# kkaytekin/Supervised-Depth-Estimation-from-Polarized-Images

Measured on AMD Instinct MI355X. Metric: train images/sec (512x612, 3-encoder), higher is better.
Workload: dtype f32; 1 GPU; BASELINE configs[2]: full 3-encoder (augment_xolp+augment_normals), multi-scale loss scales=[0,1,2,3], batch 16 per GPU, 512x612 frames (network/loss on 512x640 padded), dropout 0.1, Adam lr 1e-4, fp32; global_batch=16, height=512, width=640, frame_width=612, parallelism=dp1

## Files before the change

### include/polardepth.h

```cpp
#ifndef POLARDEPTH_H
#define POLARDEPTH_H

#include <stddef.h>
#include <stdint.h>

#ifdef __cplusplus
extern "C" {
#endif

#define PD_OK 0
#define PD_EINVAL (-22)
#define PD_ELAUNCH (-5)

const char* pd_last_error(void);
int pd_version(void);

#define PD_POLAR_LS 0
#define PD_POLAR_STOKES 1
#define PD_POLAR_PRECISE_NORMALS 1
#define PD_POLAR_IEEE_RHO 2
#define PD_POLAR_NT_LOADS 4
#define PD_POLAR_PLAIN_LOADS 8

size_t pd_polar_tables_bytes(int n_d, int n_s1, int n_s2);
int pd_polar_tables_pack(const double* x_d, const double* y_d, int n_d,
                         const double* x_s1, const double* y_s1, int n_s1,
                         const double* x_s2, const double* y_s2, int n_s2,
                         void* host_blob, size_t blob_bytes);
int pd_polar_tables_build(double n, void* host_blob, size_t blob_bytes, size_t* blob_bytes_used);

int pd_polar_fwd(const void* pol, const void* mask, void* xolp, void* xolp_std, void* normals,
                 void* ints, const void* tables, size_t tables_bytes,
                 int B, int H, int W, int Wout, int mode, int flags, void* stream);

int pd_polar_normals_from_xolp(const void* xolp, void* normals, const void* tables, size_t tables_bytes,
                               int B, int H, int W, int flags, void* stream);

int pd_polar_calc_normals(const void* phi, const void* theta, void* out, int B, long P, int phi_f64, int theta_f64,
                          void* stream);

int pd_polar_theta(const void* rho, void* theta_d, void* theta_s1, void* theta_s2, void* bins,
                   const void* tables, size_t tables_bytes, long n, void* stream);

int pd_polar_fit_matrix(const double angles_rad[4], double coef_out[12]);

#define PD_POLAR_U8 0
#define PD_POLAR_U16 1
#define PD_POLAR_F32 2
int pd_polar_general_fwd(const void* pol, int dtype, const double* coef, void* iun, void* xolp, void* xolp_std,
                         void* normals, const void* tables, size_t tables_bytes,
                         int B, int H, int W, int Wout, int flags, void* stream);

#define PD_XOLP_STATS_BYTES 4184
size_t pd_xolp_stats_workspace(int B, int H, int W);
int pd_xolp_stats(const void* xolp, const void* mask, void* stats, void* workspace, size_t ws_bytes,
                  int B, int H, int W, int ld, const float thresholds[2], int accumulate, void* stream);

#define PD_CONV_AUTO 0u
#define PD_CONV_FP32_MFMA 1u
#define PD_CONV_BF16X3 2u
#define PD_CONV_WGRAD_SPLIT_IN_REGS 4u
#define PD_CONV_GENERAL_KERNELS 8u
#define PD_CONV_X3_IM2COL 16u
#define PD_CONV_WGRAD_ROW_WORKGROUPS 32u
#define PD_CONV_BF16 128u
#define PD_CONV_FLAGS_ALL 191u
int pd_conv2d_tile_m(long M, int Cout);
long pd_conv2d_stats_rows(long M, int Cout);
int pd_conv2d_uses_x3(long M, int Cout, int C, int KH, int KW, int stride, int pad, int mode, int act, int has_out_scale,
                      int Ho, int Wo, unsigned flags);
int pd_conv2d_uses_bf16(long M, int Cout, int C, int KH, int KW, int stride, int pad, int mode, int act, int has_out_scale,
                        int Ho, int Wo, unsigned flags);
int pd_conv2d_route(long M, int Cout, int C, int KH, int KW, int stride, int pad, int mode, int act, int has_out_scale,
                    int Ho, int Wo, unsigned flags);
int pd_conv2d(const void* x, const void* w, const void* bias, const void* out_scale, void* y, void* stats,
              int N, int H, int W, int C, long sN, long sH, long sW, long sC,
              int Ho, int Wo, int Cout, int KH, int KW, int stride, int pad, int mode, int act,
              int affine, float sub, float div, long ldy, unsigned flags, void* stream);

int pd_conv16(const void* x, const void* w, const void* bias, void* y, int N, int H, int W, int C,
              long sN, long sH, long sW, int Ho, int Wo, int Cout, long ldy, int mode, int act, void* stream);

size_t pd_conv16_wgrad_workspace(int C);
int pd_conv16_wgrad(const void* x, const void* dz, void* dw, void* dbias, void* workspace, size_t ws_bytes,
                    int N, int H, int W, int C, long sN, long sH, long sW, long ldd, int accumulate, void* stream);

int pd_dgrad_s2_filters(const void* wt, void* wsub, int Cin, int Cout, void* stream);
int pd_conv2d_rect(const void* x, const void* w, void* y, int N, int H, int W, int C, long sN, long sH, long sW, long sC,
                   int Ho, int Wo, int Cout, int KH, int KW, int pad_h, int pad_w, int mode, long ldy, unsigned flags,
                   void* stream);
int pd_interleave4(const void* sub, void* dx, int N, int Ho, int Wo, int C, void* stream);

int pd_conv2d_add(const void* x, const void* w, const void* addend, long ld_add, void* y,
                  int N, int H, int W, int C, long sN, long sH, long sW, long sC,
                  int Ho, int Wo, int Cout, int KH, int KW, int stride, int pad, int mode, long ldy, unsigned flags,
                  void* stream);

size_t pd_conv2d_wgrad_workspace(long M, int Cout, int K, unsigned flags);
int pd_conv2d_wgrad(const void* x, const void* dy, void* dw, void* dbias, void* workspace, size_t ws_bytes,
                    int N, int H, int W, int C, long sN, long sH, long sW, long sC,
                    int Ho, int Wo, int Cout, int KH, int KW, int stride, int pad, int mode,
                    int affine, float sub, float div, long ldd, int accumulate, unsigned flags, void* stream);
int pd_conv2d_wgrad_uses_x3(long M, int Cout, int C, int KH, int KW, int stride, int pad, int mode, int H, int W, int Ho, int Wo,
                            unsigned flags);
int pd_conv2d_wgrad_uses_bf16(long M, int Cout, int C, int KH, int KW, int stride, int pad, int mode, int H, int W, int Ho, int Wo,
                              unsigned flags);

int pd_stem_s2d_input(const void* x, void* out, int N, int C, int H, int W, long sN, long sC, long sH, long sW,
                      int affine, float sub, float div, void* stream);
int pd_stem_s2d_weight(const void* w, void* w2, int Cout, int C, void* stream);
int pd_stem_s2d_weight_grad(const void* dw2, void* dw, int Cout, int C, int accumulate, void* stream);

int pd_weight_transpose(const void* w, void* wt, int Cout, int T, int Cin, void* stream);
int pd_weight_transpose_batched(const void* src, void* dst, const void* table, const void* blk, int n, int nblocks,
                                void* stream);

int pd_bn_fwd_finalize(const void* partial, long R, int C, double count, const void* gamma, const void* beta,
                       void* running_mean, void* running_var, float momentum, float eps, void* acc_ws, long acc_len,
                       void* scale, void* shift, void* save_mean, void* save_invstd, int training, void* stream);
int pd_bn_bwd_finalize(const void* partial, long R, int C, double count, void* acc_ws, long acc_len, void* dgamma,
                       void* dbeta, void* coef, int accumulate, void* stream);
long pd_chain_bwd_rows(int N, int H, int W, int C);
int pd_chain_fwd(const void* x, const void* scale, const void* shift, const void* res, void* out,
                 int N, int H, int W, int C, long ld_res, long ld_out, int relu_pre, int pool,
                 float drop_p, uint64_t seed, uint64_t offset, const void* step_state, int relu_post, void* stream);
int pd_chain_bwd_reduce(const void* dy, long ld_dy, const void* x, const void* out, long ld_out,
                        const void* scale, const void* shift, const void* mean, const void* invstd,
                        void* partial, int N, int H, int W, int C, int relu_pre, int pool, float drop_p,
                        uint64_t seed, uint64_t offset, const void* step_state, int relu_post, void* stream);
int pd_chain_bwd_apply(const void* dy, long ld_dy, const void* x, const void* out, long ld_out,
                       const void* scale, const void* shift, const void* mean, const void* invstd,
                       const void* coef, void* dx, void* dres, int N, int H, int W, int C, int relu_pre,
                       int pool, float drop_p, uint64_t seed, uint64_t offset, const void* step_state, int relu_post,
                       void* stream);

int pd_maxpool3s2_fwd(const void* x, void* y, void* idx, int N, int H, int W, int C, void* stream);
int pd_maxpool3s2_bwd(const void* idx, const void* dy, void* dx, int N, int H, int W, int C, void* stream);
int pd_maxpool3s2_bwd_add(const void* idx, const void* dy, const void* addend, long ld_add, void* dx, int N, int H, int W,
                          int C, void* stream);

int pd_upcat_fwd(const void* a, const void* skip, long ld_skip, void* out, int N, int H, int W, int Ca, int Cs,
                 void* stream);
int pd_up_bwd(const void* dout, long ld_d, void* da, int N, int H, int W, int Ca, void* stream);
int pd_up_bwd_elu(const void* dout, long ld_d, const void* elu_y, void* da, int N, int H, int W, int Ca, void* stream);

int pd_up2x_ac_fwd(const void* a, void* out, int N, int H, int W, int C, void* stream);
int pd_up2x_ac_bwd(const void* dout, void* da, int N, int H, int W, int C, void* stream);
int pd_relu_add(const void* x, const void* res, void* out, long n, int relu, void* stream);

// ... 139 lines not shown
```

### supervised-depth-estimation-from-polarized-images_amd/csrc/conv.hip

```cpp
#include "pd_common.h"
#include <cstdlib>
#include <type_traits>

namespace {

typedef float f32x16 __attribute__((ext_vector_type(16)));
typedef unsigned int u32x4 __attribute__((ext_vector_type(4)));

constexpr int BK = 32;
constexpr int LDT = BK;
constexpr int NT = 256;
constexpr unsigned OOB = 0x80000000u;

enum { MODE_ZERO = 0, MODE_REFLECT = 1, MODE_TRANSPOSED = 2 };
enum { ACT_NONE = 0, ACT_RELU = 1, ACT_ELU = 2, ACT_SIGMOID = 3 };

#define PD_I(n) std::integral_constant<int, n>{}
#define PD_SB __builtin_amdgcn_sched_barrier(0);

template <typename F> void with_mode(int mode, F&& f) {
    if (mode == MODE_ZERO) f(PD_I(MODE_ZERO)); else if (mode == MODE_REFLECT) f(PD_I(MODE_REFLECT)); else f(PD_I(MODE_TRANSPOSED));
}
template <typename F> void with_bool(bool b, F&& f) { if (b) f(std::true_type{}); else f(std::false_type{}); }

// ... 1980 lines not shown
        auto mm = [&](const x3::Terms& t, auto g_tag, auto n_tag) {
            constexpr int G = decltype(g_tag)::value, N = decltype(n_tag)::value, T = N / 2, BLK = N % 2;
            const unsigned* bv = T < 3 ? t.h : T < 5 ? t.m : t.l;
            const u32x4 av = T == 0 ? fa[G][BLK][0] : T == 1 ? fa[G][BLK][1] : T == 2 ? fa[G][BLK][2] : T == 3 ? fa[G][BLK][0] : T == 4 ? fa[G][BLK][1] : fa[G][BLK][0];
            acc[BLK] = __builtin_amdgcn_mfma_f32_32x32x16_bf16(bf(av), bf(u32x4{bv[0], bv[1], bv[2], bv[3]}), acc[BLK], 0, 0, 0);
        };
        x3::sp_h<0>(x0, t0); x3::sp_h<1>(x0, t0); x3::sp_h<2>(x0, t0); x3::sp_h<3>(x0, t0);
        PD_SB
#define PD_XP(j) if constexpr (SPREAD) load_x_piece(nxt, PD_I(j));
#define PD_DP(j) if constexpr (SPREAD) load_d_piece(buf_tag, PD_I(j));
        mm(t0, PD_I(0), PD_I(0)); x3::sp_m<0>(x0, t0); PD_XP(0) PD_SB
        mm(t0, PD_I(0), PD_I(1)); x3::sp_m<1>(x0, t0); PD_XP(1) PD_SB
        mm(t0, PD_I(0), PD_I(2)); x3::sp_m<2>(x0, t0); PD_XP(2) PD_SB
        mm(t0, PD_I(0), PD_I(3)); x3::sp_m<3>(x0, t0); PD_XP(3) PD_SB
        mm(t0, PD_I(0), PD_I(4)); x3::sp_h<0>(dv, td); x3::sp_h<1>(dv, td); x3::sp_h<2>(dv, td); x3::sp_h<3>(dv, td); PD_DP(0) PD_SB
        mm(t0, PD_I(0), PD_I(5)); x3::sp_m<0>(dv, td); PD_DP(1) PD_SB
#undef PD_XP
#undef PD_DP
        mm(t0, PD_I(0), PD_I(6)); x3::sp_l<0>(t0); x3::sp_h<0>(x1, t1); PD_SB
        mm(t0, PD_I(0), PD_I(7)); x3::sp_l<1>(t0); x3::sp_h<1>(x1, t1); PD_SB
        mm(t0, PD_I(0), PD_I(8)); x3::sp_l<2>(t0); x3::sp_h<2>(x1, t1); PD_SB
        mm(t0, PD_I(0), PD_I(9)); x3::sp_l<3>(t0); x3::sp_h<3>(x1, t1); PD_SB
        mm(t0, PD_I(0), PD_I(10)); x3::sp_m<1>(dv, td); PD_SB
        mm(t0, PD_I(0), PD_I(11)); x3::sp_m<2>(dv, td); PD_SB
        mm(t1, PD_I(1), PD_I(0)); x3::sp_m<0>(x1, t1); PD_SB
        mm(t1, PD_I(1), PD_I(1)); x3::sp_m<1>(x1, t1); PD_SB
        mm(t1, PD_I(1), PD_I(2)); x3::sp_m<2>(x1, t1); PD_SB
        mm(t1, PD_I(1), PD_I(3)); x3::sp_m<3>(x1, t1); PD_SB
        mm(t1, PD_I(1), PD_I(4)); x3::sp_m<3>(dv, td); PD_SB
        mm(t1, PD_I(1), PD_I(5)); x3::sp_l<0>(td); x3::sp_l<1>(td); PD_SB
        mm(t1, PD_I(1), PD_I(6)); x3::sp_l<0>(t1); PD_SB
        mm(t1, PD_I(1), PD_I(7)); x3::sp_l<1>(t1); PD_SB
        mm(t1, PD_I(1), PD_I(8)); x3::sp_l<2>(t1); PD_SB
        mm(t1, PD_I(1), PD_I(9)); x3::sp_l<3>(t1); PD_SB
        mm(t1, PD_I(1), PD_I(10)); x3::sp_l<2>(td); x3::sp_l<3>(td); PD_SB
        mm(t1, PD_I(1), PD_I(11));
        if constexpr (BIAS) bsum += ((dv[0] + dv[1]) + (dv[2] + dv[3])) + ((dv[4] + dv[5]) + (dv[6] + dv[7]));
        *reinterpret_cast<u32x4*>(lds_c + sp_off + (NXT * P_BYTES + 0 * 4096u)) = u32x4{td.h[0], td.h[1], td.h[2], td.h[3]};
        *reinterpret_cast<u32x4*>(lds_c + sp_off + (NXT * P_BYTES + 1 * 4096u)) = u32x4{td.m[0], td.m[1], td.m[2], td.m[3]};
        *reinterpret_cast<u32x4*>(lds_c + sp_off + (NXT * P_BYTES + 2 * 4096u)) = u32x4{td.l[0], td.l[1], td.l[2], td.l[3]};
        dma_wait();
        __syncthreads();
    };

    {
        const std::integral_constant<unsigned, 0> d0{};
        const std::integral_constant<unsigned, 1> d1{};
        load_x_all(d0);
        load_d(d0);
        load_d(d1);
        dma_wait();
        __syncthreads();
        split_d(d0);
        __syncthreads();
    }
    for (int q = 0; q < nchunks; q += 2) {
        chunk(std::integral_constant<unsigned, 0>{});
        if (q + 1 < nchunks) chunk(std::integral_constant<unsigned, 1>{});
        if ((q & (FLUSH - 2)) == FLUSH - 2) flush();
    }
    flush();

#pragma unroll
    for (int blk = 0; blk < 2; ++blk) {
        const int k = k0 + wave * 32 + fi;
#pragma unroll
        for (int r = 0; r < 16; ++r) {
            const int co = co0 + 32 * blk + (r & 3) + 8 * (r >> 2) + 4 * fk;
            if (co < a.Co && k < a.K) a.part[((long)s * a.Co + co) * a.K + k] = acc_sum[blk][r];
        }
    }
    if constexpr (BIAS) {
        if (do_bias) {
            float* red = smem_all;
            red[wave * 64 + lane] = bsum;
            __syncthreads();
            if (tid < 64 && co0 + tid < a.Co) a.bpart[(long)s * a.Co + co0 + tid] = (red[tid] + red[64 + tid]) + (red[128 + tid] + red[192 + tid]);
        }
    }
}

#include "conv_wgrad_halo.hpp"
#include "conv_wgrad_roll.hpp"

__global__ __launch_bounds__(256) void reduce_rows_kernel(const float* __restrict__ part, float* __restrict__ out,
                                                          int S, long n, int accumulate) {
    __shared__ float red[4][64];
    const int col = threadIdx.x & 63, sl = threadIdx.x >> 6;
    const long i = blockIdx.x * 64L + col;
    float a0 = 0.f, a1 = 0.f, a2 = 0.f, a3 = 0.f;
    if (i < n) {
        int j = sl;
        for (; j + 12 < S; j += 16) {
            a0 += part[(long)j * n + i];
            a1 += part[(long)(j + 4) * n + i];
            a2 += part[(long)(j + 8) * n + i];
            a3 += part[(long)(j + 12) * n + i];
        }
        for (; j < S; j += 4) a0 += part[(long)j * n + i];
    }
    red[sl][col] = (a0 + a1) + (a2 + a3);
    __syncthreads();
    if (sl == 0 && i < n) {
        const float s = (red[0][col] + red[1][col]) + (red[2][col] + red[3][col]);
        out[i] = accumulate ? out[i] + s : s;
    }
}

__global__ __launch_bounds__(256) void weight_transpose_kernel(const float* __restrict__ w, float* __restrict__ wt,
                                                               int Co, int T, int Ci) {
    const long n = (long)Co * T * Ci;
    for (long i = blockIdx.x * 256L + threadIdx.x; i < n; i += (long)gridDim.x * 256) {
        const int co = (int)(i % Co);
        const long r = i / Co;
        const int t = (int)(r % T);
        const int ci = (int)(r / T);
        wt[i] = w[((long)co * T + t) * Ci + ci];
    }
}

__global__ __launch_bounds__(256) void weight_transpose_batched_kernel(const float* __restrict__ src, float* __restrict__ dst,
                                                                       const int* __restrict__ table,
                                                                       const int* __restrict__ blk, int n) {
    __shared__ float tile[32][33];
    int lo = 0, hi = n;
    while (hi - lo > 1) {
        const int mid = (lo + hi) >> 1;
        if (blk[mid] <= (int)blockIdx.x) lo = mid; else hi = mid;
    }
    const int off = table[4 * lo], Co = table[4 * lo + 1], T = table[4 * lo + 2], Ci = table[4 * lo + 3];
    const float* w = src + off;
    float* wt = dst + off;
    int lb = (int)blockIdx.x - blk[lo];
    const int tiles_ci = (Ci + 31) >> 5, tiles_co = (Co + 31) >> 5;
    const int ci0 = (lb % tiles_ci) << 5; lb /= tiles_ci;
    const int co0 = (lb % tiles_co) << 5;
    const int t = lb / tiles_co;
    const int x = threadIdx.x & 31, y = threadIdx.x >> 5;
#pragma unroll
    for (int r = y; r < 32; r += 8)
        if (co0 + r < Co && ci0 + x < Ci) tile[r][x] = w[((long)(co0 + r) * T + t) * Ci + ci0 + x];
    __syncthreads();
#pragma unroll
    for (int r = y; r < 32; r += 8)
        if (ci0 + r < Ci && co0 + x < Co) wt[((long)(ci0 + r) * T + t) * Co + co0 + x] = tile[x][r];
}

inline int wgrad_tco(int Co) { return Co > 32 ? 64 : (Co > 16 ? 32 : 16); }

inline bool wgrad_x3c_enabled(unsigned flags) { return !(flags & (PD_CONV_FP32_MFMA | PD_CONV_WGRAD_SPLIT_IN_REGS)); }
inline bool wgrad_x3_on(unsigned flags) { return (flags & PD_CONV_WGRAD_SPLIT_IN_REGS) && !(flags & PD_CONV_FP32_MFMA); }

void wgrad_plan(long M, int Co, int K, unsigned flags, int* S, long* mper) {
    const int tco = wgrad_tco(Co);
    const long tiles = (long)((Co + tco - 1) / tco) * ((K + WG_K - 1) / WG_K);
    const bool x3c = tco == 64 && wgrad_x3c_enabled(flags) && !(flags & PD_CONV_GENERAL_KERNELS);
    const long total = x3c ? (512 / tiles < 4 ? 1536 : M >= (1L << 20) ? 1024 : 512) : (tiles <= 32 ? 768 : 1536);
    long s = total / tiles;
    const long smax = (M + 511) / 512;
    if (s > smax) s = smax;
    if (s < 1) s = 1;
    long per = (M + s - 1) / s;
    per = (per + WG_MC - 1) / WG_MC * WG_MC;
    s = (M + per - 1) / per;
    if (s < 1) s = 1;
    *S = (int)s; *mper = per;
}

enum WgradFamily { WGRAD_GENERAL = 0, WGRAD_UNI, WGRAD_UNI_X3, WGRAD_X3C, WGRAD_HALO, WGRAD_ROLL };
struct WgradRoute {
    int family;
    int tco, S; long mper;
    bool vec, row8;
    int nb, nbw;
    int s_cap; bool bf16;
    WgradRollPlan roll;
};

static WgradRoute route_wgrad(const WgradArgs& a, bool vec, unsigned flags, size_t ws_bytes) {
    WgradRoute r{};
    r.vec = vec; r.tco = wgrad_tco(a.Co);
    wgrad_plan(a.M, a.Co, a.K, flags, &r.S, &r.mper);
    const bool refl_ok = a.mode == MODE_REFLECT && a.pad == 1 && a.KH == 3 && a.KW == 3 && a.stride == 1 && a.Ho == a.H && a.Wo == a.W && a.H >= 3;
    if (!(a.mode == MODE_ZERO || refl_ok)) return r;
    if (wgrad_x3c_enabled(flags) && !(flags & (PD_CONV_GENERAL_KERNELS | PD_CONV_X3_IM2COL)) && wgrad_halo_eligible(a, vec)) {
        r.bf16 = (flags & PD_CONV_BF16) != 0;
        const size_t per_slice = ((size_t)a.Co * a.K + a.Co) * sizeof(float);
        r.s_cap = (int)std::min<size_t>((r.bf16 ? pd_conv2d_wgrad_workspace(a.M, a.Co, a.K, flags) : ws_bytes) / per_slice, 1 << 20);
        r.family = !(flags & PD_CONV_WGRAD_ROW_WORKGROUPS) && wgrad_roll_eligible(a, vec, r.s_cap, r.roll) ? WGRAD_ROLL : WGRAD_HALO;
        return r;
    }
    r.nb = (a.pad + a.stride - 1) / a.stride; r.nbw = (r.nb + 1) / 2;
    if (!(flags & PD_CONV_GENERAL_KERNELS) && (r.tco == 64 || r.tco == 32) && vec && a.Co % 4 == 0 && a.Wo % 2 == 0 && a.ldd % 4 == 0 &&
        a.Ho >= 2 * r.nb && a.Wo >= 4 * r.nbw && a.Wo >= 14 && (2 * r.nb + 1) * (2 * r.nbw + 1) <= 31 && r.mper % WG_MC == 0 &&
        a.M % 4 == 0 && a.K >= 4) {
        r.family = r.tco == 32 ? WGRAD_UNI : wgrad_x3c_enabled(flags) ? WGRAD_X3C : wgrad_x3_on(flags) ? WGRAD_UNI_X3 : WGRAD_UNI;
        r.row8 = a.Wo % 8 == 0 && r.mper % 8 == 0 && a.M % 8 == 0;
    }
    return r;
}

static int launch_wgrad_slices(const WgradArgs& a, const WgradRoute& r, bool bias, hipStream_t st) {
    const dim3 grid((unsigned)(((long)a.ktiles * a.ctiles * a.S + 7) / 8 * 8)), block(NT);
    const bool reflect = a.mode == MODE_REFLECT;
    if (r.family == WGRAD_GENERAL) {
        const auto gen = [&](auto tco) { with_bool(r.vec, [&](auto v) { with_bool(reflect, [&](auto refl) {
            hipLaunchKernelGGL((conv_wgrad_kernel<decltype(tco)::value, decltype(v)::value, decltype(refl)::value ? MODE_REFLECT : MODE_ZERO>), grid, block, 0, st, a);
        }); }); };
        if (r.tco == 64) gen(PD_I(64)); else if (r.tco == 32) gen(PD_I(32)); else gen(PD_I(16));
        return PD_OK;
    }
    WgradUniArgs ua; ua.g = a; ua.nb = r.nb; ua.nbw = r.nbw;
    if (r.family == WGRAD_X3C) {
        static const hipError_t lds_ok = [] {
            hipError_t e = hipSuccess;
            for (const void* f : {reinterpret_cast<const void*>(conv_wgrad_x3c_kernel<true, true>), reinterpret_cast<const void*>(conv_wgrad_x3c_kernel<false, true>),
                                  reinterpret_cast<const void*>(conv_wgrad_x3c_kernel<true, false>), reinterpret_cast<const void*>(conv_wgrad_x3c_kernel<false, false>),
                                  reinterpret_cast<const void*>(conv_wgrad_x3c_kernel<true, false, true>), reinterpret_cast<const void*>(conv_wgrad_x3c_kernel<false, false, true>)}) {
                const hipError_t rc = hipFuncSetAttribute(f, hipFuncAttributeMaxDynamicSharedMemorySize, x3c::LDS_BYTES);
                if (rc != hipSuccess) e = rc;
            }
            return e;
        }();
        PD_REQUIRE(lds_ok == hipSuccess, "pd_conv2d_wgrad: cannot reserve %u bytes of LDS", x3c::LDS_BYTES);
        with_bool(bias, [&](auto b) {
            constexpr bool B = decltype(b)::value;
            if (reflect) hipLaunchKernelGGL((conv_wgrad_x3c_kernel<B, false, true>), grid, block, x3c::LDS_BYTES, st, ua);
            else if (r.row8) hipLaunchKernelGGL((conv_wgrad_x3c_kernel<B, true>), grid, block, x3c::LDS_BYTES, st, ua);
            else hipLaunchKernelGGL((conv_wgrad_x3c_kernel<B, false>), grid, block, x3c::LDS_BYTES, st, ua);
        });
    } else if (r.tco == 32) {
        with_bool(reflect, [&](auto refl) { hipLaunchKernelGGL((conv_wgrad_uni_kernel<decltype(refl)::value, true, 32>), grid, block, 0, st, ua); });
    } else {
        with_bool(reflect, [&](auto refl) { with_bool(bias, [&](auto b) {
            constexpr bool R = decltype(refl)::value, B = decltype(b)::value;
            if (r.family == WGRAD_UNI_X3) hipLaunchKernelGGL((conv_wgrad_uni_kernel<R, B, 64, true>), grid, block, 0, st, ua);
            else hipLaunchKernelGGL((conv_wgrad_uni_kernel<R, B>), grid, block, 0, st, ua);
        }); });
    }
    return PD_OK;
}

static void fill_wgrad_args(WgradArgs& a, int N, int H, int W, int C, long sN, long sH, long sW, long sC, int Ho, int Wo, int Co,
                            int KH, int KW, int stride, int pad, int mode, int affine, float sub, float div, long ldd) {
    a.N = N; a.H = H; a.W = W; a.C = C; a.sN = sN; a.sH = sH; a.sW = sW; a.sC = sC;
    a.Ho = Ho; a.Wo = Wo; a.Co = Co; a.KH = KH; a.KW = KW; a.stride = stride; a.pad = pad; a.mode = mode;
    a.affine = affine; a.sub = sub; a.div = div;
    a.K = KH * KW * C; a.M = (long)N * Ho * Wo; a.ldd = ldd;
}

}

extern "C" size_t pd_conv2d_wgrad_workspace(long M, int Co, int K, unsigned flags) {
    int S; long mper;
    wgrad_plan(M, Co, K, flags, &S, &mper);
    if (wgrad_x3c_enabled(flags) && !(flags & (PD_CONV_GENERAL_KERNELS | PD_CONV_X3_IM2COL))) {
        const int sh = std::max(wgrad_halo_slices_bound(Co, K), wgrad_roll_slices_bound(Co, K));
        const long cap = (M + 63) / 64;
        S = S > (sh < cap ? sh : (int)cap) ? S : (sh < cap ? sh : (int)cap);
    }
    return ((size_t)S * Co * K + (size_t)S * Co) * sizeof(float);
}

extern "C" int pd_conv2d_wgrad_uses_x3(long M, int Co, int C, int KH, int KW, int stride, int pad, int mode, int H, int W, int Ho,
                                       int Wo, unsigned flags) {
    if (Ho <= 0 || Wo <= 0) return 0;
    WgradArgs a{};
    fill_wgrad_args(a, (int)(M / ((long)Ho * Wo)), H, W, C, (long)H * W * C, (long)W * C, C, 1, Ho, Wo, Co, KH, KW, stride, pad, mode,
                    0, 0.f, 1.f, Co);
    a.M = M;
    const int family = route_wgrad(a, vec16_ok(a.x, C, a.sN, a.sH, a.sW, a.sC, a.affine), flags, pd_conv2d_wgrad_workspace(M, Co, a.K, flags)).family;
    return family == WGRAD_ROLL ? 3 : family == WGRAD_HALO ? 2 : family == WGRAD_X3C ? 1 : 0;
}

extern "C" int pd_conv2d_wgrad_uses_bf16(long M, int Co, int C, int KH, int KW, int stride, int pad, int mode, int H, int W, int Ho,
                                         int Wo, unsigned flags) {
    if (!(flags & PD_CONV_BF16) || !pd::conv_flags_ok(flags)) return 0;
    const int r = pd_conv2d_wgrad_uses_x3(M, Co, C, KH, KW, stride, pad, mode, H, W, Ho, Wo, flags);
    return r >= 2 ? r : 0;
}

extern "C" int pd_conv2d_wgrad(const void* x, const void* dy, void* dw, void* dbias, void* workspace, size_t ws_bytes,
                               int N, int H, int W, int C, long sN, long sH, long sW, long sC,
                               int Ho, int Wo, int Co, int KH, int KW, int stride, int pad, int mode,
                               int affine, float sub, float div, long ldd, int accumulate, unsigned flags, void* stream) {
    PD_REQUIRE(x && dy && dw && workspace, "pd_conv2d_wgrad: null tensor");
    PD_REQUIRE(pd::conv_flags_ok(flags), "pd_conv2d_wgrad: bad flags 0x%x", flags);
    PD_REQUIRE(mode == MODE_ZERO || mode == MODE_REFLECT, "pd_conv2d_wgrad: mode must be 0 or 1");
    PD_REQUIRE(Ho <= (H + 2 * pad - KH) / stride + 1 && Wo <= (W + 2 * pad - KW) / stride + 1,
               "pd_conv2d_wgrad: output grid does not match input/filter geometry");
    PD_REQUIRE(ldd >= Co && (ldd % 4 == 0 || Co < 4) , "pd_conv2d_wgrad: bad dy row stride");
    if (N == 0) return PD_OK;
    WgradArgs a;
    a.x = (const float*)x; a.dy = (const float*)dy;
    fill_wgrad_args(a, N, H, W, C, sN, sH, sW, sC, Ho, Wo, Co, KH, KW, stride, pad, mode, affine, sub, div, ldd);
    const size_t need = pd_conv2d_wgrad_workspace(a.M, Co, a.K, flags);
    PD_REQUIRE(ws_bytes >= need, "pd_conv2d_wgrad: workspace too small (%zu < %zu)", ws_bytes, need);
    PD_REQUIRE(pd::aligned16(dy) && (ldd % 4 == 0 || Co < 4), "pd_conv2d_wgrad: dy must be 16-byte aligned rows");
    const WgradRoute r = route_wgrad(a, vec16_ok(x, C, sN, sH, sW, sC, affine), flags, ws_bytes);
    a.S = r.S; a.mper = r.mper;
    PD_REQUIRE(a.mper * ldd * 4 < 0x7fffffffL, "pd_conv2d_wgrad: slice too large for 32-bit offsets");
    PD_REQUIRE((a.mper / ((long)Ho * Wo) + 2) * sN * 4 < 0x7fffffffL, "pd_conv2d_wgrad: image too large for 32-bit offsets");
    a.part = (float*)workspace;
    a.bpart = dbias ? a.part + (size_t)a.S * Co * a.K : nullptr;
    a.ktiles = (a.K + WG_K - 1) / WG_K; a.ctiles = (Co + r.tco - 1) / r.tco;
    hipStream_t st = (hipStream_t)stream;
    int S = a.S;
    if (r.family == WGRAD_ROLL) S = launch_wgrad_roll(a, r.roll, st, dbias != nullptr, r.bf16);
    else if (r.family == WGRAD_HALO) S = launch_wgrad_halo(a, r.s_cap, st, dbias != nullptr, r.bf16);
    else if (int rc = launch_wgrad_slices(a, r, dbias != nullptr, st)) return rc;
    a.bpart = dbias ? a.part + (size_t)S * Co * a.K : nullptr;
    if (int rc = pd::check_launch("pd_conv2d_wgrad")) return rc;
    const long nw = (long)Co * a.K;
    hipLaunchKernelGGL(reduce_rows_kernel, dim3((unsigned)((nw + 63) / 64)), dim3(256), 0, st, a.part, (float*)dw, S, nw, accumulate);
    if (dbias)
        hipLaunchKernelGGL(reduce_rows_kernel, dim3((unsigned)((Co + 63) / 64)), dim3(256), 0, st, a.bpart, (float*)dbias, S, (long)Co, accumulate);
    return pd::check_launch("pd_conv2d_wgrad/reduce");
}

extern "C" int pd_weight_transpose(const void* w, void* wt, int Co, int T, int Ci, void* stream) {
    PD_REQUIRE(w && wt && Co > 0 && T > 0 && Ci > 0, "pd_weight_transpose: bad arguments");
    const long n = (long)Co * T * Ci;
    const long blocks = (n + 255) / 256;
    hipLaunchKernelGGL(weight_transpose_kernel, dim3((unsigned)(blocks > 4096 ? 4096 : blocks)), dim3(256), 0,
                       (hipStream_t)stream, (const float*)w, (float*)wt, Co, T, Ci);
    return pd::check_launch("pd_weight_transpose");
}

extern "C" int pd_weight_transpose_batched(const void* src, void* dst, const void* table, const void* blk, int n,
                                           int nblocks, void* stream) {
    PD_REQUIRE(src && dst && table && blk && n > 0 && nblocks > 0, "pd_weight_transpose_batched: bad arguments");
    hipLaunchKernelGGL(weight_transpose_batched_kernel, dim3((unsigned)nblocks), dim3(256), 0, (hipStream_t)stream,
                       (const float*)src, (float*)dst, (const int*)table, (const int*)blk, n);
    return pd::check_launch("pd_weight_transpose_batched");
}

namespace {
__global__ __launch_bounds__(256) void dgrad_s2_filters_kernel(const float* __restrict__ wt, float* __restrict__ wsub,
                                                               int Ci, int Co) {
    const long cc = (long)Ci * Co, total = 9 * cc;
    for (long i = blockIdx.x * 256L + threadIdx.x; i < total; i += (long)gridDim.x * 256) {
        const int cls = i < cc ? 0 : i < 3 * cc ? 1 : i < 5 * cc ? 2 : 3, ph = cls >> 1, pw = cls & 1;
        const long base = cc * (cls == 0 ? 0 : cls == 1 ? 1 : cls == 2 ? 3 : 5);
        long r = i - base;
        const int co = (int)(r % Co); r /= Co;
        const int kw2 = pw ? (int)(r & 1) : 0; r >>= pw;
        const int kh2 = ph ? (int)(r & 1) : 0; r >>= ph;
        const int ci = (int)r;
        const int kh = ph ? (kh2 ? 2 : 0) : 1, kw = pw ? (kw2 ? 2 : 0) : 1;
        wsub[i] = wt[(((long)ci * 3 + kh) * 3 + kw) * Co + co];
    }
}
__global__ __launch_bounds__(256) void interleave4_kernel(const float* __restrict__ sub, float* __restrict__ dx, int N, int Ho,
                                                          int Wo, int C) {
    const int cq = C >> 2;
    const long per = (long)N * Ho * Wo * cq, total = 4 * per;
    for (long i = blockIdx.x * 256L + threadIdx.x; i < total; i += (long)gridDim.x * 256) {
        const int c4 = (int)(i % cq) * 4;
        long r = i / cq;
        const int pw = (int)(r & 1); r >>= 1;
        const int j = (int)(r % Wo); r /= Wo;
        const int ph = (int)(r & 1); r >>= 1;
        const int ii = (int)(r % Ho);
        const long n = r / Ho;
        const float4 v = ldg4(sub + ((long)(ph * 2 + pw) * N * Ho * Wo + (n * Ho + ii) * (long)Wo + j) * C + c4);
        *reinterpret_cast<float4*>(dx + ((n * 2 * Ho + 2 * ii + ph) * (long)(2 * Wo) + 2 * j + pw) * C + c4) = v;
    }
}
}

extern "C" int pd_dgrad_s2_filters(const void* wt, void* wsub, int Ci, int Co, void* stream) {
    PD_REQUIRE(wt && wsub && Ci > 0 && Co > 0, "pd_dgrad_s2_filters: bad arguments");
    const long total = 9L * Ci * Co, blocks = (total + 255) / 256;
    hipLaunchKernelGGL(dgrad_s2_filters_kernel, dim3((unsigned)(blocks > 2048 ? 2048 : blocks)), dim3(256), 0,
                       (hipStream_t)stream, (const float*)wt, (float*)wsub, Ci, Co);
    return pd::check_launch("pd_dgrad_s2_filters");
}

extern "C" int pd_interleave4(const void* sub, void* dx, int N, int Ho, int Wo, int C, void* stream) {
    PD_REQUIRE(sub && dx && N > 0 && Ho > 0 && Wo > 0 && C > 0 && C % 4 == 0, "pd_interleave4: bad arguments");
    const long total = 4L * N * Ho * Wo * (C / 4), blocks = (total + 255) / 256;
    hipLaunchKernelGGL(interleave4_kernel, dim3((unsigned)(blocks > 8192 ? 8192 : blocks)), dim3(256), 0,
                       (hipStream_t)stream, (const float*)sub, (float*)dx, N, Ho, Wo, C);
    return pd::check_launch("pd_interleave4");
}

namespace {

__global__ __launch_bounds__(256) void s2d_input_kernel(const float* __restrict__ x, float* __restrict__ out, int N,
                                                        int C, int H, int W, long sN, long sC, long sH, long sW,
                                                        int affine, float sub, float div) {
    const int H2 = H >> 1, W2 = W >> 1, C4 = 4 * C;
// ... 99 lines not shown
```

### supervised-depth-estimation-from-polarized-images_amd/polardepth/ops.py

```python
import os

import torch

from ._lib import lib, check, ptr, stream_ptr

MODE_ZERO, MODE_REFLECT, MODE_TRANSPOSED = 0, 1, 2
ACT_NONE, ACT_RELU, ACT_ELU, ACT_SIGMOID = 0, 1, 2, 3
CL = torch.channels_last
PROFILE = None

CONV_AUTO, CONV_FP32_MFMA, CONV_BF16X3, CONV_WGRAD_SPLIT_IN_REGS, CONV_GENERAL_KERNELS, CONV_X3_IM2COL = 0, 1, 2, 4, 8, 16
CONV_WGRAD_ROW_WORKGROUPS = 32
CONV_BF16 = 128
CONV_FLAGS = (CONV_FP32_MFMA if os.environ.get("PD_CONV_X3", "1") == "0" else
              CONV_X3_IM2COL if os.environ.get("PD_CONV_HALO", "1") == "0" else CONV_AUTO)
WGRAD_FLAGS = (CONV_FP32_MFMA if os.environ.get("PD_WGRAD_X3C", "1") == "0" else
               CONV_X3_IM2COL if os.environ.get("PD_CONV_HALO", "1") == "0" else
               CONV_WGRAD_ROW_WORKGROUPS if os.environ.get("PD_WGRAD_ROLL", "1") == "0" else CONV_AUTO)


class conv_flags:

    def __init__(self, conv=None, wgrad=None):
        self.new = (conv, wgrad)

    def __enter__(self):
        global CONV_FLAGS, WGRAD_FLAGS
        self.old = (CONV_FLAGS, WGRAD_FLAGS)
        if self.new[0] is not None:
            CONV_FLAGS = int(self.new[0])
        if self.new[1] is not None:
            WGRAD_FLAGS = int(self.new[1])
        return self

    def __exit__(self, *exc):
        global CONV_FLAGS, WGRAD_FLAGS
        CONV_FLAGS, WGRAD_FLAGS = self.old
        return False


def conv_bf16_mode():
    return (bool(CONV_FLAGS & CONV_BF16), bool(WGRAD_FLAGS & CONV_BF16))


def _with_bf16(word, bf16):
    if bf16 is None:
        return word
    if bf16 and not (word & (CONV_FP32_MFMA | CONV_BF16X3)):
        return word | CONV_BF16
    return word & ~CONV_BF16


def _profiled(label, flops, fn, shape=None):
    if PROFILE is None:
        return fn()
    e0, e1 = torch.cuda.Event(enable_timing=True), torch.cuda.Event(enable_timing=True)
    e0.record()
    r = fn()
    e1.record()
    PROFILE.append((label, flops, e0, e1, shape))
    return r


_IGEMM_LABELS = ("conv_igemm_kernel<{bm},{bn},{gather}>", "conv_igemm_uni_kernel<{bm},{bn}>", "conv_igemm_x3_kernel<{bm},{bn}>",
                 "conv_halo_x3_kernel<8x32,64>", "conv_halo_bf16_kernel<8x32,64>")


def _igemm_label(M, Co, vec, kind, C=0, KH=1, KW=1, stride=1, pad=0, mode=0, act=ACT_NONE, out_scale=False, out_hw=(0, 0),
                 flags=None):
    flags = CONV_FLAGS if flags is None else flags
    if not vec:
        flags = CONV_FP32_MFMA | CONV_GENERAL_KERNELS
    r = lib.pd_conv2d_route(M, Co, C, KH, KW, stride, pad, mode, act, int(out_scale), out_hw[0], out_hw[1], flags)
    return _IGEMM_LABELS[r & 15].format(bm=r >> 12, bn=(r >> 4) & 255, gather="vec" if vec else "scalar")


def _require_cuda(*ts):
    for t in ts:
        if t is not None and not t.is_cuda:
            raise RuntimeError("polardepth ops need CUDA(HIP) tensors; there is no CPU fallback")


def empty_nhwc(n, c, h, w, device):
    return torch.empty((n, c, h, w), dtype=torch.float32, device=device, memory_format=CL)


def is_nhwc(t):
    n, c, h, w = t.shape
    return t.stride() == (h * w * c, 1, w * c, c) or t.is_contiguous(memory_format=CL)


def as_nhwc(t):
    return t if is_nhwc(t) else t.contiguous(memory_format=CL)


def weight_cl(w):
    return w if w.is_contiguous(memory_format=CL) else w.contiguous(memory_format=CL)


def conv_out_size(h, k, s, p):
    return (h + 2 * p - k) // s + 1
# ... 300 lines not shown
```

Baseline: 351.2 images/s.

## Add dedicated halo-tiled bf16x3 weight-gradient kernel for 4x4 stem convolutions

Adds a specialized weight-gradient kernel for stride-1, pad-2, 4x4 convolutions with 8/12/36 input channels, the shape of the encoder stems. It stages dy tiles and halo row windows of x in LDS as three-way bf16 splits, double-buffered, with the next tile's global loads interleaved between the MFMA groups. The goal is to avoid the im2col-style generic X3C path for these small-C layers and its poor reuse. The kernel is selected automatically, can be turned off with an environment flag, and brings its own slice planning and LDS attribute setup.

```diff
diff --git a/include/polardepth.h b/include/polardepth.h
--- a/include/polardepth.h
+++ b/include/polardepth.h
@@ -64,7 +64,8 @@
 #define PD_CONV_X3_IM2COL 16u
 #define PD_CONV_WGRAD_ROW_WORKGROUPS 32u
 #define PD_CONV_BF16 128u
-#define PD_CONV_FLAGS_ALL 191u
+#define PD_CONV_WGRAD_NO_STEM 256u
+#define PD_CONV_FLAGS_ALL 447u
 int pd_conv2d_tile_m(long M, int Cout);
 long pd_conv2d_stats_rows(long M, int Cout);
 int pd_conv2d_uses_x3(long M, int Cout, int C, int KH, int KW, int stride, int pad, int mode, int act, int has_out_scale,
diff --git a/supervised-depth-estimation-from-polarized-images_amd/csrc/conv.hip b/supervised-depth-estimation-from-polarized-images_amd/csrc/conv.hip
--- a/supervised-depth-estimation-from-polarized-images_amd/csrc/conv.hip
+++ b/supervised-depth-estimation-from-polarized-images_amd/csrc/conv.hip
@@ -2086,6 +2086,7 @@
 
 #include "conv_wgrad_halo.hpp"
 #include "conv_wgrad_roll.hpp"
+#include "conv_wgrad_stem.hpp"
 
 __global__ __launch_bounds__(256) void reduce_rows_kernel(const float* __restrict__ part, float* __restrict__ out,
                                                           int S, long n, int accumulate) {
@@ -2171,7 +2172,7 @@
     *S = (int)s; *mper = per;
 }
 
-enum WgradFamily { WGRAD_GENERAL = 0, WGRAD_UNI, WGRAD_UNI_X3, WGRAD_X3C, WGRAD_HALO, WGRAD_ROLL };
+enum WgradFamily { WGRAD_GENERAL = 0, WGRAD_UNI, WGRAD_UNI_X3, WGRAD_X3C, WGRAD_HALO, WGRAD_ROLL, WGRAD_STEM };
 struct WgradRoute {
     int family;
     int tco, S; long mper;
@@ -2179,6 +2180,7 @@
     int nb, nbw;
     int s_cap; bool bf16;
     WgradRollPlan roll;
+    int s_ws;
 };
 
 static WgradRoute route_wgrad(const WgradArgs& a, bool vec, unsigned flags, size_t ws_bytes) {
@@ -2200,6 +2202,11 @@
         a.M % 4 == 0 && a.K >= 4) {
         r.family = r.tco == 32 ? WGRAD_UNI : wgrad_x3c_enabled(flags) ? WGRAD_X3C : wgrad_x3_on(flags) ? WGRAD_UNI_X3 : WGRAD_UNI;
         r.row8 = a.Wo % 8 == 0 && r.mper % 8 == 0 && a.M % 8 == 0;
+        if (r.family == WGRAD_X3C && !(flags & (PD_CONV_WGRAD_NO_STEM | PD_CONV_X3_IM2COL | PD_CONV_BF16)) && wgrad_stem_eligible(a, vec)) {
+            const size_t per_slice = ((size_t)a.Co * a.K + a.Co) * sizeof(float);
+            r.family = WGRAD_STEM;
+            r.s_ws = (int)std::min<size_t>(pd_conv2d_wgrad_workspace(a.M, a.Co, a.K, flags) / per_slice, 1 << 20);
+        }
     }
     return r;
 }
@@ -2274,7 +2281,7 @@
                     0, 0.f, 1.f, Co);
     a.M = M;
     const int family = route_wgrad(a, vec16_ok(a.x, C, a.sN, a.sH, a.sW, a.sC, a.affine), flags, pd_conv2d_wgrad_workspace(M, Co, a.K, flags)).family;
-    return family == WGRAD_ROLL ? 3 : family == WGRAD_HALO ? 2 : family == WGRAD_X3C ? 1 : 0;
+    return family == WGRAD_ROLL ? 3 : family == WGRAD_HALO ? 2 : (family == WGRAD_X3C || family == WGRAD_STEM) ? 1 : 0;
 }
 
 extern "C" int pd_conv2d_wgrad_uses_bf16(long M, int Co, int C, int KH, int KW, int stride, int pad, int mode, int H, int W, int Ho,
@@ -2312,6 +2319,10 @@
     int S = a.S;
     if (r.family == WGRAD_ROLL) S = launch_wgrad_roll(a, r.roll, st, dbias != nullptr, r.bf16);
     else if (r.family == WGRAD_HALO) S = launch_wgrad_halo(a, r.s_cap, st, dbias != nullptr, r.bf16);
+    else if (r.family == WGRAD_STEM) {
+        S = launch_wgrad_stem(a, r.s_ws, st, dbias != nullptr);
+        PD_REQUIRE(S > 0, "pd_conv2d_wgrad: cannot reserve the LDS of conv_wgrad_stem_x3_kernel");
+    }
     else if (int rc = launch_wgrad_slices(a, r, dbias != nullptr, st)) return rc;
     a.bpart = dbias ? a.part + (size_t)S * Co * a.K : nullptr;
     if (int rc = pd::check_launch("pd_conv2d_wgrad")) return rc;
diff --git a/supervised-depth-estimation-from-polarized-images_amd/csrc/conv_wgrad_stem.hpp b/supervised-depth-estimation-from-polarized-images_amd/csrc/conv_wgrad_stem.hpp
--- /dev/null
+++ b/supervised-depth-estimation-from-polarized-images_amd/csrc/conv_wgrad_stem.hpp
@@ -0,0 +1,259 @@
+namespace wgs {
+template <int C, int TR> struct Geo {
+    static constexpr int NJ = C / 4;
+    static constexpr int NPX = 32 * TR;
+    static constexpr int XR = TR + 3;
+    static constexpr int XQ = 35 * C / 4;
+    static constexpr int NXI = XR * XQ;
+    static constexpr int NIX = (NXI + NT - 1) / NT;
+    static constexpr unsigned ROWB = 35 * C * 2;
+    static constexpr unsigned DPL = NPX * 64, XPL = XR * ROWB;
+    static constexpr unsigned DP_BYTES = 3 * DPL, XP_BYTES = (3 * XPL + 15) / 16 * 16;
+    static constexpr unsigned BUF_BYTES = DP_BYTES + XP_BYTES;
+    static constexpr unsigned LDS_BYTES = 2 * BUF_BYTES;
+    static constexpr int WGS_PER_CU = LDS_BYTES > 53 * 1024 ? 2 : 3;
+    static_assert(C % 4 == 0 && (4 * C) % 16 == 0 && ROWB % 8 == 0 && XPL % 8 == 0, "row-window geometry");
+    static_assert(NT * 16 <= LDS_BYTES, "the bias reduction reuses the planes");
+};
+typedef float f32x4 __attribute__((ext_vector_type(4)));
+}
+
+struct WgradStemArgs {
+    WgradArgs g;
+    int tiles_w, tiles_h, ntiles_total, tiles_per_slice;
+};
+
+template <int C, int TR, bool BIAS>
+__global__ __launch_bounds__(NT, (wgs::Geo<C, TR>::WGS_PER_CU)) void conv_wgrad_stem_x3_kernel(const WgradStemArgs sa) {
+    using namespace wgs;
+    using wgh::lds_char; using wgh::tr_read;
+    using G = Geo<C, TR>;
+    constexpr int NJ = G::NJ, XQ = G::XQ, NXI = G::NXI, NIX = G::NIX, ND = TR, NITEMS = ND + NIX;
+    constexpr unsigned ROWB = G::ROWB, DPL = G::DPL, XPL = G::XPL, DP_BYTES = G::DP_BYTES, BUF_BYTES = G::BUF_BYTES;
+    static_assert(NITEMS <= TR * NJ, "one item of the next tile behind every column group");
+    const WgradArgs& a = sa.g;
+    extern __shared__ __attribute__((aligned(16))) float smem_all[];
+    char* lds_c = reinterpret_cast<char*>(smem_all);
+
+    const int tid = threadIdx.x, lane = tid & 63;
+    const int kh = __builtin_amdgcn_readfirstlane(tid >> 6);
+    const int nwg = a.ctiles * a.S;
+    int b = ((int)blockIdx.x & 7) * ((int)gridDim.x >> 3) + ((int)blockIdx.x >> 3);
+    if (b >= nwg) return;
+    const int cob = b % a.ctiles;
+    const int s = b / a.ctiles;
+    const int co0 = cob * 32;
+    const int t_beg = s * sa.tiles_per_slice;
+    const int t_end = min(t_beg + sa.tiles_per_slice, sa.ntiles_total);
+
+    unsigned d_voff[ND];
+#pragma unroll
+    for (int i = 0; i < ND; ++i) d_voff[i] = (unsigned)((i * a.Wo + (tid >> 3)) * (int)a.ldd + co0 + 4 * (tid & 7)) * 4u;
+    const unsigned d_dst = (unsigned)((tid >> 3) * 64 + (tid & 7) * 8);
+    int x_r[NIX], x_e[NIX]; unsigned x_dst[NIX];
+#pragma unroll
+    for (int i = 0; i < NIX; ++i) {
+        const int e = tid + NT * i;
+        x_r[i] = e / XQ; x_e[i] = 4 * (e - x_r[i] * XQ);
+        x_dst[i] = DP_BYTES + (unsigned)x_r[i] * ROWB + 2u * (unsigned)x_e[i];
+    }
+    const bool x_last_ok = tid + NT * (NIX - 1) < NXI;
+    const int row_len = a.W * C;
+
+    int l_t = t_beg, l_n, l_ty, l_tx;
+    {
+        const int per_img = sa.tiles_h * sa.tiles_w;
+        l_n = t_beg / per_img;
+        const int rem = t_beg - l_n * per_img;
+        l_ty = rem / sa.tiles_w; l_tx = rem - l_ty * sa.tiles_w;
+        l_n = __builtin_amdgcn_readfirstlane(l_n); l_ty = __builtin_amdgcn_readfirstlane(l_ty); l_tx = __builtin_amdgcn_readfirstlane(l_tx);
+    }
+    __amdgpu_buffer_rsrc_t rd, rx;
+    int l_iy0 = 0, l_e0 = 0;
+    auto tile_begin = [&]() {
+        const int oy0 = l_ty * TR, ox0 = l_tx * 32;
+        const long pix0 = ((long)l_n * a.Ho + oy0) * a.Wo + ox0;
+        const bool live = l_t < t_end;
+        rd = make_rsrc(a.dy + pix0 * a.ldd, live ? (unsigned)(((long)(TR - 1) * a.Wo + 32) * a.ldd * 4) : 0u);
+        rx = make_rsrc(a.x + (long)l_n * a.sN, live ? (unsigned)((long)a.sN * 4) : 0u);
+        l_iy0 = oy0 - 2; l_e0 = (ox0 - 2) * C;
+    };
+    auto tile_next = [&]() {
+        ++l_t;
+        if (++l_tx == sa.tiles_w) { l_tx = 0; if (++l_ty == sa.tiles_h) { l_ty = 0; ++l_n; } }
+    };
+    float4 dv[ND], xv[NIX];
+    auto load_d = [&](auto i_tag) { constexpr int I = decltype(i_tag)::value; dv[I] = buf_ld4(rd, d_voff[I]); };
+    auto load_x = [&](auto i_tag) {
+        constexpr int I = decltype(i_tag)::value;
+        const int iy = l_iy0 + x_r[I], e = l_e0 + x_e[I];
+        const bool ok = (unsigned)iy < (unsigned)a.H && (unsigned)e < (unsigned)row_len && (I < NIX - 1 || x_last_ok);
+        xv[I] = buf_ld4(rx, ok ? (unsigned)(iy * (int)a.sH + e) * 4u : OOB);
+    };
+    const unsigned dsign = (s & 1) ? 0x80008000u : 0u;
+    float4 bs4 = make_float4(0.f, 0.f, 0.f, 0.f);
+    const bool do_bias = BIAS && a.bpart != nullptr;
+    auto put3 = [&](const float4 v, unsigned off, unsigned plane_stride, unsigned sg) {
+        uint2 h, m, l;
+        x3::split2(v.x, v.y, h.x, m.x, l.x);
+        x3::split2(v.z, v.w, h.y, m.y, l.y);
+        *reinterpret_cast<uint2*>(lds_c + off) = uint2{h.x ^ sg, h.y ^ sg};
+        *reinterpret_cast<uint2*>(lds_c + off + plane_stride) = uint2{m.x ^ sg, m.y ^ sg};
+        *reinterpret_cast<uint2*>(lds_c + off + 2 * plane_stride) = uint2{l.x ^ sg, l.y ^ sg};
+    };
+    auto item = [&](auto dst_tag, auto k_tag) {
+        constexpr unsigned DST = decltype(dst_tag)::value;
+        constexpr int K = decltype(k_tag)::value;
+        if constexpr (K < ND) {
+            put3(dv[K], DST * BUF_BYTES + d_dst + 2048u * K, DPL, dsign);
+            if constexpr (BIAS) { if (do_bias) { bs4.x += dv[K].x; bs4.y += dv[K].y; bs4.z += dv[K].z; bs4.w += dv[K].w; } }
+            load_d(k_tag);
+        } else if constexpr (K < NITEMS) {
+            constexpr int I = K - ND;
+            if (I < NIX - 1 || x_last_ok) put3(xv[I], DST * BUF_BYTES + x_dst[I], XPL, 0u);
+            load_x(std::integral_constant<int, I>{});
+        }
+    };
+    auto items_all = [&](auto dst_tag) {
+        item(dst_tag, PD_I(0)); item(dst_tag, PD_I(1)); item(dst_tag, PD_I(2)); item(dst_tag, PD_I(3));
+        item(dst_tag, PD_I(4)); item(dst_tag, PD_I(5)); item(dst_tag, PD_I(6)); item(dst_tag, PD_I(7));
+    };
+    static_assert(NITEMS <= 8, "items_all");
+
+    const int fg = lane >> 4, fq = (lane & 15) >> 2, fp = lane & 3;
+    lds_char* const lds_a = (lds_char*)lds_c + (unsigned)((8 * fg + fq) * 64 + 8 * fp);
+    lds_char* const lds_b = (lds_char*)lds_c + (DP_BYTES + (unsigned)kh * ROWB + 2u * (unsigned)((8 * fg + fq) * C + 4 * fp));
+
+    f32x4 acc[2][NJ];
+#pragma unroll
+    for (int cb = 0; cb < 2; ++cb)
+#pragma unroll
+        for (int j = 0; j < NJ; ++j) acc[cb][j] = f32x4{0.f, 0.f, 0.f, 0.f};
+    auto bf = [](uint2 lo, uint2 hi) { return __builtin_bit_cast(x3::bf16x8, u32x4{lo.x, lo.y, hi.x, hi.y}); };
+
+#define PD_U(n) std::integral_constant<unsigned, n>{}
+    tile_begin();
+    load_d(PD_I(0)); if constexpr (ND > 1) load_d(PD_I(1));
+    load_x(PD_I(0)); if constexpr (NIX > 1) load_x(PD_I(1)); if constexpr (NIX > 2) load_x(PD_I(2));
+    if constexpr (NIX > 3) load_x(PD_I(3)); if constexpr (NIX > 4) load_x(PD_I(4));
+    static_assert(ND <= 2 && NIX <= 5, "prologue");
+    tile_next(); tile_begin();
+    items_all(PD_U(0));
+    tile_next(); tile_begin();
+    __syncthreads();
+
+    auto tile = [&](auto buf_tag) {
+        constexpr unsigned BUF = decltype(buf_tag)::value;
+        const std::integral_constant<unsigned, BUF ^ 1> nxt{};
+#pragma unroll
+        for (int ks = 0; ks < TR; ++ks) {
+            x3::bf16x8 fa[2][3];
+#pragma unroll
+            for (int cb = 0; cb < 2; ++cb)
+#pragma unroll
+                for (int tm = 0; tm < 3; ++tm) {
+                    const unsigned o = BUF * BUF_BYTES + (unsigned)(tm * DPL + ks * 2048 + cb * 32);
+                    fa[cb][tm] = bf(tr_read(lds_a, o), tr_read(lds_a, o + 4 * 64));
+                }
+#pragma unroll
+            for (int jg = 0; jg < NJ; ++jg) {
+                x3::bf16x8 fb[3];
+#pragma unroll
+                for (int tm = 0; tm < 3; ++tm) {
+                    const unsigned o = BUF * BUF_BYTES + (unsigned)(tm * XPL + ks * ROWB + jg * 32);
+                    fb[tm] = bf(tr_read(lds_b, o), tr_read(lds_b, o + 4 * C * 2));
+                }
+#pragma unroll
+                for (int pr = 0; pr < 6; ++pr) {
+                    const int ta = pr == 0 ? 0 : pr == 1 ? 0 : pr == 2 ? 1 : pr == 3 ? 0 : pr == 4 ? 1 : 2;
+                    const int tb = pr == 0 ? 0 : pr == 1 ? 1 : pr == 2 ? 0 : pr == 3 ? 2 : pr == 4 ? 1 : 0;
+#pragma unroll
+                    for (int cb = 0; cb < 2; ++cb)
+                        acc[cb][jg] = __builtin_amdgcn_mfma_f32_16x16x32_bf16(fa[cb][ta], fb[tb], acc[cb][jg], 0, 0, 0);
+                }
+                const int g = ks * NJ + jg;
+                if (g == 0) item(nxt, PD_I(0));
+                else if (g == 1) item(nxt, PD_I(1));
+                else if (g == 2) item(nxt, PD_I(2));
+                else if (g == 3) item(nxt, PD_I(3));
+                else if (g == 4) item(nxt, PD_I(4));
+                else if (g == 5) item(nxt, PD_I(5));
+                else if (g == 6) item(nxt, PD_I(6));
+                else if (g == 7) item(nxt, PD_I(7));
+            }
+        }
+        tile_next(); tile_begin();
+        __syncthreads();
+    };
+    for (int t = t_beg; t < t_end; t += 2) {
+        tile(PD_U(0));
+        if (t + 1 < t_end) tile(PD_U(1));
+    }
+#undef PD_U
+
+#pragma unroll
+    for (int cb = 0; cb < 2; ++cb)
+#pragma unroll
+        for (int jg = 0; jg < NJ; ++jg) {
+            const long k = (long)kh * (4 * C) + 16 * jg + (lane & 15);
+#pragma unroll
+            for (int r = 0; r < 4; ++r) {
+                const int co = co0 + 16 * cb + 4 * fg + r;
+                a.part[((long)s * a.Co + co) * a.K + k] = dsign ? -acc[cb][jg][r] : acc[cb][jg][r];
+            }
+        }
+    if constexpr (BIAS) {
+        if (do_bias) {
+            float4* red = reinterpret_cast<float4*>(smem_all);
+            red[tid] = bs4;
+            __syncthreads();
+            if (tid < 32) {
+                const int q4 = tid >> 2, e = tid & 3;
+                float sum = 0.f;
+                for (int j = 0; j < 32; ++j) sum += reinterpret_cast<const float*>(&red[j * 8 + q4])[e];
+                a.bpart[(long)s * a.Co + co0 + tid] = sum;
+            }
+        }
+    }
+}
+
+static int wgrad_stem_tr(int C) { return C == 36 ? 1 : 2; }
+static bool wgrad_stem_eligible(const WgradArgs& a, bool vec) {
+    return vec && a.mode == MODE_ZERO && a.KH == 4 && a.KW == 4 && a.stride == 1 && a.pad == 2 && a.Ho == a.H && a.Wo == a.W &&
+           a.Co % 64 == 0 && (a.C == 36 || a.C == 12 || a.C == 8) && a.sW == a.C && a.sC == 1 && a.Wo % 32 == 0 &&
+           a.Ho % wgrad_stem_tr(a.C) == 0 && a.ldd % 4 == 0 && a.M == (long)a.N * a.Ho * a.Wo &&
+           (long)a.sN * 4 < 0x7fffffffL && ((long)a.Wo + 32) * a.ldd * 4 < 0x7fffffffL;
+}
+static void wgrad_stem_plan(const WgradArgs& a, int s_ws, WgradStemArgs& sa) {
+    const int tr = wgrad_stem_tr(a.C);
+    sa.tiles_w = a.Wo / 32; sa.tiles_h = a.Ho / tr;
+    sa.ntiles_total = a.N * sa.tiles_h * sa.tiles_w;
+    int S = 256 * (tr == 1 ? 2 : 3) / (a.Co / 32);
+    if (S > s_ws) S = s_ws;
+    if (S > sa.ntiles_total) S = sa.ntiles_total;
+    if (S < 1) S = 1;
+    sa.tiles_per_slice = (sa.ntiles_total + S - 1) / S;
+    sa.g.S = (sa.ntiles_total + sa.tiles_per_slice - 1) / sa.tiles_per_slice;
+}
+
+static int launch_wgrad_stem(WgradArgs a, int s_ws, hipStream_t st, bool bias) {
+    WgradStemArgs sa;
+    a.ctiles = a.Co / 32;
+    sa.g = a;
+    wgrad_stem_plan(a, s_ws, sa);
+    const int S = sa.g.S;
+    if (a.bpart) sa.g.bpart = a.part + (size_t)S * a.Co * a.K;
+    const long nwg = (long)a.ctiles * S;
+    const dim3 grid((unsigned)((nwg + 7) / 8 * 8)), block(NT);
+    hipError_t rc = hipSuccess;
+    auto go = [&](auto c_tag, auto tr_tag) { with_bool(bias, [&](auto bt) {
+        constexpr int CV = decltype(c_tag)::value, TRV = decltype(tr_tag)::value;
+        constexpr unsigned LDS = wgs::Geo<CV, TRV>::LDS_BYTES;
+        auto* const f = conv_wgrad_stem_x3_kernel<CV, TRV, decltype(bt)::value>;
+        static const hipError_t lds_ok = hipFuncSetAttribute(reinterpret_cast<const void*>(f), hipFuncAttributeMaxDynamicSharedMemorySize, LDS);
+        rc = lds_ok;
+        if (rc == hipSuccess) hipLaunchKernelGGL(f, grid, block, LDS, st, sa);
+    }); };
+    if (a.C == 36) go(PD_I(36), PD_I(1)); else if (a.C == 12) go(PD_I(12), PD_I(2)); else go(PD_I(8), PD_I(2));
+    return rc == hipSuccess ? S : -1;
+}
diff --git a/supervised-depth-estimation-from-polarized-images_amd/polardepth/ops.py b/supervised-depth-estimation-from-polarized-images_amd/polardepth/ops.py
--- a/supervised-depth-estimation-from-polarized-images_amd/polardepth/ops.py
+++ b/supervised-depth-estimation-from-polarized-images_amd/polardepth/ops.py
@@ -11,12 +11,15 @@
 
 CONV_AUTO, CONV_FP32_MFMA, CONV_BF16X3, CONV_WGRAD_SPLIT_IN_REGS, CONV_GENERAL_KERNELS, CONV_X3_IM2COL = 0, 1, 2, 4, 8, 16
 CONV_WGRAD_ROW_WORKGROUPS = 32
+CONV_WGRAD_NO_STEM = 256
 CONV_BF16 = 128
 CONV_FLAGS = (CONV_FP32_MFMA if os.environ.get("PD_CONV_X3", "1") == "0" else
               CONV_X3_IM2COL if os.environ.get("PD_CONV_HALO", "1") == "0" else CONV_AUTO)
 WGRAD_FLAGS = (CONV_FP32_MFMA if os.environ.get("PD_WGRAD_X3C", "1") == "0" else
                CONV_X3_IM2COL if os.environ.get("PD_CONV_HALO", "1") == "0" else
                CONV_WGRAD_ROW_WORKGROUPS if os.environ.get("PD_WGRAD_ROLL", "1") == "0" else CONV_AUTO)
+if os.environ.get("PD_WGRAD_STEM", "1") == "0":
+    WGRAD_FLAGS |= CONV_WGRAD_NO_STEM
 
 
 class conv_flags:
```

Result: no change. 353.8 images/s, median of 6 (+0.7%).
